# jyjblrd/Low-Cost-Mocap

Measured on AMD Instinct MI355X. Metric: triangulated 3D markers/sec at 8 cams x 16 markers, higher is better.
Workload: dtype f64

## Files before the change

### low-cost-mocap_amd/csrc/capi.hip

```cpp
#include <hip/hip_runtime.h>

#include <cmath>
#include <cstdarg>
#include <cstdio>
#include <cstdlib>
#include <cstring>
#include <mutex>
#include <string>
#include <vector>

#include "../../include/mocap_core.h"
#include "ctx.hpp"

using namespace mocap;

int mocap_ctx::fail(int code, const char* fmt, ...) {
  char buf[512];
  va_list ap;
  va_start(ap, fmt);
  vsnprintf(buf, sizeof buf, fmt, ap);
  va_end(ap);
  {
    std::lock_guard<std::mutex> lk(err_mu);
    err = buf;
// ... 29 lines not shown
  cap = want;
  return 0;
}

hipError_t PinBuf::reserve(size_t need, size_t want, unsigned flags) {
  if (need <= cap) return hipSuccess;
  if (ptr) (void)hipHostFree(ptr);
  ptr = nullptr;
  cap = 0;
  const hipError_t e = hipHostMalloc(&ptr, want, flags);
  if (e == hipSuccess) cap = want;
  return e;
}

int spin_wait(mocap_ctx* ctx, Event& event) {
  HIP_TRY(ctx, event.ready());
  HIP_TRY(ctx, hipEventRecord(event.ev, ctx->stream));
  for (long spins = 0;; spins++) {
    const hipError_t e = hipEventQuery(event.ev);
    if (e == hipSuccess) return MOCAP_OK;
    if (e != hipErrorNotReady) return ctx->hip_fail(e, "hipEventQuery");
    if (spins > 2000000) {
      HIP_TRY(ctx, hipStreamSynchronize(ctx->stream));
      return MOCAP_OK;
    }
  }
}

extern "C" int mocap_create(int device_id, mocap_ctx** out) {
  if (!out) return MOCAP_E_ARG;
  *out = nullptr;
  int ndev = 0;
  if (hipGetDeviceCount(&ndev) != hipSuccess || device_id < 0 || device_id >= ndev) return MOCAP_E_HIP;
  mocap_ctx* c = new mocap_ctx();
  c->device = device_id;
  if (hipSetDevice(device_id) != hipSuccess || hipStreamCreate(&c->own_stream) != hipSuccess) {
    delete c;
    return MOCAP_E_HIP;
  }
  c->stream = c->own_stream;
  hipDeviceProp_t prop;
  if (hipGetDeviceProperties(&prop, device_id) == hipSuccess) c->num_cus = prop.multiProcessorCount;
  const char* t = getenv("MOCAP_FRAME_THREADS");
  if (t) {
    int v = atoi(t);
    if (v == 64 || v == 128 || v == 256) c->frame_threads = v;
  }
  if ((t = getenv("MOCAP_HEAVY_THRESHOLD"))) c->heavy_threshold = atoi(t);
  if ((t = getenv("MOCAP_SLICE_SIZE"))) c->slice_size = atoi(t);
  if ((t = getenv("MOCAP_FORCE_WIDE"))) c->force_wide = atoi(t) ? 1 : 0;
  if ((t = getenv("MOCAP_PRUNE"))) c->prune = atoi(t) ? 1 : 0;
  if ((t = getenv("MOCAP_EIGCUT"))) c->eigcut = atoi(t) ? 1 : 0;
  if ((t = getenv("MOCAP_EVAL_BB"))) c->eval_bb = atoi(t) ? 1 : 0;
  if ((t = getenv("MOCAP_BB_PL")) && atoi(t) >= 1 && atoi(t) <= 64) c->bb_pl = atoi(t);
  if ((t = getenv("MOCAP_BB_FLUSH")) && atoi(t) >= 1) c->bb_flush = atoi(t);
  if ((t = getenv("MOCAP_BB_MIN_G")) && atoi(t) >= 0) c->bb_min_g = atoi(t);
  if ((t = getenv("MOCAP_FRAME_LAUNCHES"))) c->frame_launches = atoi(t) == 3 ? 3 : 1;
  *out = c;
  return MOCAP_OK;
}

extern "C" void mocap_destroy(mocap_ctx* ctx) {
  if (!ctx) return;
  (void)hipSetDevice(ctx->device);
  (void)hipStreamSynchronize(ctx->stream);
  if (ctx->own_stream) (void)hipStreamDestroy(ctx->own_stream);
  delete ctx;
}

extern "C" const char* mocap_last_error(const mocap_ctx* ctx) {
  if (!ctx) return "null context";
  static thread_local std::string mine;
  {
    std::lock_guard<std::mutex> lk(const_cast<mocap_ctx*>(ctx)->err_mu);
    mine = ctx->err;
  }
  return mine.c_str();
}
extern "C" const char* mocap_version(void) { return "mocap_core 0.1 (gfx950)"; }

extern "C" int mocap_set_stream(mocap_ctx* ctx, void* hip_stream) {
  if (!ctx) return MOCAP_E_ARG;
  std::lock_guard<std::mutex> lk(ctx->mu);
  hipStream_t ns = hip_stream ? (hipStream_t)hip_stream : ctx->own_stream;
  if (ns != ctx->stream && ctx->dev_outstanding) {
    int prev_dev = -1;
    (void)hipGetDevice(&prev_dev);
    HIP_TRY(ctx, hipSetDevice(ctx->device));
    const hipError_t e = hipStreamWaitEvent(ns, ctx->handover_event.ev, 0);
    if (prev_dev >= 0 && prev_dev != ctx->device) (void)hipSetDevice(prev_dev);
    if (e != hipSuccess) return ctx->hip_fail(e, "hipStreamWaitEvent(handover)");
    ctx->frame_q_dirty();
  }
  ctx->stream = ns;
  return MOCAP_OK;
}

extern "C" const char* mocap_last_frame_kernel(mocap_ctx* ctx) {
  if (!ctx) return "none";
  std::lock_guard<std::mutex> lk(ctx->mu);
  return ctx->last_frame_kernel;
}

extern "C" int mocap_synchronize(mocap_ctx* ctx) {
  if (!ctx) return MOCAP_E_ARG;
  std::lock_guard<std::mutex> lk(ctx->mu);
  HIP_TRY(ctx, hipSetDevice(ctx->device));
// ... 413 lines not shown
```

### low-cost-mocap_amd/csrc/ctx.hpp

```cpp
#pragma once
#include <hip/hip_runtime.h>

#include <mutex>
#include <string>
#include <vector>

#include "kernels.hpp"

#define HIP_TRY(ctx, expr)                                     \
  do {                                                         \
    hipError_t e__ = (expr);                                   \
    if (e__ != hipSuccess) return (ctx)->hip_fail(e__, #expr); \
  } while (0)

struct Owned {
  Owned() = default;
  Owned(const Owned&) = delete;
};

struct DevBuf : Owned {
  void* ptr = nullptr;
  size_t cap = 0;
  int reserve(size_t bytes);
  ~DevBuf() { if (ptr) (void)hipFree(ptr); }
};

struct PinBuf : Owned {
  void* ptr = nullptr;
  size_t cap = 0;
  hipError_t reserve(size_t need, size_t want, unsigned flags);
  ~PinBuf() { if (ptr) (void)hipHostFree(ptr); }
};

struct Event : Owned {
  hipEvent_t ev = nullptr;
  hipError_t ready() { return ev ? hipSuccess : hipEventCreateWithFlags(&ev, hipEventDisableTiming); }
  ~Event() { if (ev) (void)hipEventDestroy(ev); }
};

struct Carver {
  uintptr_t base;
  size_t align, off = 0;
  explicit Carver(void* b, size_t align_ = 256) : base((uintptr_t)b), align(align_) {}
  template <class T>
  static size_t padded(size_t count, size_t align = 256) { return (sizeof(T) * count + align - 1) / align * align; }
  template <class T>
  T* take(size_t count) {
    T* p = (T*)(base + off);
    off += padded<T>(count, align);
    return p;
  }
  void align_to(size_t a) { off = (off + a - 1) / a * a; }
};

struct mocap_ctx {
  int device = 0;
  int num_cus = 256;
  int frame_threads = 0;
  int heavy_threshold = -1;
  int slice_size = 0;
  int hit_cap = 32;
  int force_wide = 0;
  int32_t frame_gen = 0;
  int frame_q_cap[2] = {0, 0};
  const char* last_frame_kernel = "none";
  bool frame_q_clean[2] = {false, false};
  void frame_q_dirty() { frame_q_clean[0] = frame_q_clean[1] = false; }
  int frame_launches = 1;
  int prune = 1;
  int exhaustive = 0;
  int eval_bb = 1;
  int bb_pl = 16;
  int bb_min_g = 0;
  int bb_flush = 0;
  int eigcut = 1;
  double eig_c0[3] = {0, 0, 0};
  double p3max2c = 0.0;
  double p3max2 = 0.0;
  hipStream_t own_stream = nullptr, stream = nullptr;
  Event handover_event;
  bool dev_outstanding = false;
  int mark_enqueued();
  std::mutex mu;
  std::string err;
  std::mutex err_mu;
  uint32_t flags = 1u;
  int C = 0;
  std::vector<double> hK, hR, ht, hF;
  DevBuf tables;
  const double* d_K9 = nullptr;
  mocap::CamView cv{};
  PinBuf ba_pin;
  Event ba_event;
  PinBuf ba_stage;
  void (*ba_progress)(const double* x, int n, void* user) = nullptr;
  void* ba_progress_user = nullptr;
  DevBuf ba_fused;
  double ba_stamp = 0.0;
  PinBuf live_pin;
  Event live_event;
  DevBuf world;
  bool world_on = false;
  int img_C = 0, img_rows = 0, img_cols = 0, img_S = 0, img_ay = 0;
  DevBuf img_map, img_rot, img_mask, img_stage, img_tiles, img_lens, img_fix, img_fixidx, img_act, img_box, img_zero;
  int img_n_lt = 0;
  int blob_skip_dark = 1;
  int centroid_mode = 0;
  DevBuf img_grey, img_bbox;
  DevBuf compact_ws;
  DevBuf frame_ws;
  DevBuf bb_ws;
  DevBuf live_stage;
  DevBuf resub;
  DevBuf resub_ctr;
  DevBuf resub_q;
  DevBuf heavy_recs;
  DevBuf heavy_ws;
  DevBuf heavy_enum;
  uint32_t resub_calls = 0;
  DevBuf scratch[4];
  int objf_D = 0, objf_B = 0;
  float objf_q = 0.f, objf_r = 0.f;
  DevBuf objf_state;
  DevBuf objf_ws;
  uint32_t objf_calls = 0;
// ... 59 lines not shown
```

### low-cost-mocap_amd/csrc/frame_bb.hip

```cpp
#include "mocap_device.hpp"
#include "kernels.hpp"
#include <cstdlib>
#include "frame_common.hpp"

namespace mocap {

constexpr int kBBThreads = 256;
constexpr int kBBWaves = kBBThreads / 64;
constexpr int kBBRecs = kBBThreads + 64;
constexpr int bb_cw(int C) { return C <= 8 ? 1 : 2; }
constexpr uint32_t bb_rec_bytes(int CW) { return 24u + 8u * (uint32_t)CW; }

constexpr int bb_wg_per_cu(int RL) { return RL == 48 ? 5 : 4; }
constexpr int kBBLdsSlack = 1024;
struct BBLayout {
  size_t bxy, bxy_nx, cnt_nx, bt, rbound, seedkey, slot_key, claimw, recs, rpk, scr, scr_bytes, goff, gcnt, outslot, boff, bnb, seedgh, slot_g, cnt,
      misc, bpl, nh, hits, act, root_blob, root_cam, nact, bnl, bv, bcache, bpk, total;
  int ncache;
  __host__ __device__ static size_t al(size_t x, size_t a) { return (x + a - 1) / a * a; }
  __host__ __device__ BBLayout(int C, int M, int R, int CW, int wg_per_cu) {
    size_t o = 0;
    auto take = [&](size_t bytes, size_t a) {
      o = al(o, a);
      const size_t at = o;
      o += bytes;
      return at;
    };
    bxy = take(sizeof(float2) * (size_t)C * M, 16);
    bxy_nx = take(sizeof(float2) * (size_t)C * M, 16);
    cnt_nx = take(4 * (size_t)C, 4);
    bt = take(sizeof(double) * 10 * ((size_t)C * M + 1), 16);
    rbound = take(8 * (size_t)R, 8);
    claimw = take(8 * (size_t)C, 8);
    scr = seedkey = take(8 * (size_t)R, 8);
    slot_key = take(8 * (size_t)kBBWaves * R, 8);
    recs = take(8 * (size_t)kBBRecs, 8);
    rpk = take(8 * (size_t)kBBRecs * CW, 8);
    seedgh = take(4 * (size_t)R, 4);
    slot_g = take(4 * (size_t)kBBWaves * R, 4);
    scr_bytes = o - scr;
    goff = take(4 * (size_t)(R + 1), 4);
    gcnt = take(4 * (size_t)R, 4);
    outslot = take(4 * (size_t)R, 4);
    boff = take(4 * (size_t)(R + 1), 4);
    bnb = take(4 * (size_t)R, 4);
    cnt = take(4 * (size_t)C, 4);
    misc = take(4 * 16, 4);
    bpl = take(2 * (size_t)R, 2);
    nh = take((size_t)R * C, 1);
    hits = take((size_t)R * C * M, 1);
    act = take((size_t)R * C, 1);
    root_blob = take((size_t)R, 1);
    root_cam = take((size_t)R, 1);
    nact = take((size_t)R, 1);
    bnl = take((size_t)R, 1);
    bv = take((size_t)R, 1);
    bcache = take(0, 8);
    ncache = 0;
    const size_t per_entry = 8 + 8 * (size_t)CW;
    for (int per_cu = wg_per_cu; per_cu >= 1; per_cu--) {
      const size_t lim = ((size_t)160 * 1024 / per_cu - kBBLdsSlack) / 256 * 256;
      if (lim >= o + per_entry * 64) {
        const size_t n = (lim - o) / per_entry;
        ncache = (int)(n > 1024 ? 1024 : n);
        break;
      }
    }
    o += 8 * (size_t)ncache;
    bpk = o;
    o += 8 * (size_t)CW * ncache;
    total = al(o, 16);
  }
};

static int bb_fixed_slots(int C, int M, int R) {
  const char* e = getenv("MOCAP_BB_FIXED_LAYOUT");
  if (e && e[0] == '0') return 0;
  if (C == 8 && M == 16 && R <= 48) return 48;
  if (C == 8 && M == 16 && R <= 64) return 64;
  return 0;
}
static int frame_bb_root_slots(int C, int M, int R) {
  const int f = bb_fixed_slots(C, M, R);
  return f ? f : R;
}
size_t frame_bb_lds_bytes(int C, int M, int R) { return BBLayout(C, M, frame_bb_root_slots(C, M, R), bb_cw(C), bb_wg_per_cu(bb_fixed_slots(C, M, R))).total; }
static size_t frame_bb_lds_bytes_min(int C, int M, int R) {
  const BBLayout L(C, M, frame_bb_root_slots(C, M, R), bb_cw(C), bb_wg_per_cu(bb_fixed_slots(C, M, R)));
  return L.total - (8 + 8 * (size_t)bb_cw(C)) * (size_t)L.ncache;
}
bool frame_bb_fits(int C, int M, int R) {
  return C >= 2 && C <= 16 && M >= 1 && M <= 64 && R >= 1 && R <= 255 && frame_bb_lds_bytes_min(C, M, R) <= (size_t)128 * 1024;
}

template <int CW>
struct Packed {
  unsigned long long w[CW];
  __device__ __forceinline__ void clear() {
#pragma unroll
    for (int k = 0; k < CW; k++) w[k] = ~0ull;
  }
  __device__ __forceinline__ void set(int c, uint32_t idx) {
    if (CW == 1)
      w[0] ^= (unsigned long long)(idx ^ 0xFFu) << (8 * c);
    else
      w[c >> 3] ^= (unsigned long long)(idx ^ 0xFFu) << (8 * (c & 7));
  }
  __device__ __forceinline__ uint32_t get(int c) const {
    return CW == 1 ? (uint32_t)(w[0] >> (8 * c)) & 0xFFu : (uint32_t)(w[c >> 3] >> (8 * (c & 7))) & 0xFFu;
  }
};

template <int CT, bool PERK = false>
struct BBCamTables {
  const double* base;
  static constexpr int C = CT;
  static constexpr int kPq = PERK ? 12 * CT * CT : 12 * CT;
  __device__ __forceinline__ ctab_t pq(size_t off) const { return as_ctab(base + off); }
  __device__ __forceinline__ ctab_t rt(size_t off) const { return as_ctab(base + kPq + off); }
  __device__ __forceinline__ ctab_t k4(size_t off) const { return as_ctab(base + kPq + 12 * CT + off); }
  __device__ __forceinline__ const double* f() const { return base + kPq + 16 * CT; }
};
template <bool PERK>
struct BBCamTables<0, PERK> {
  const double* base;
  int C;
  __device__ __forceinline__ ctab_t pq(size_t off) const { return as_ctab(base + off); }
  __device__ __forceinline__ ctab_t rt(size_t off) const { return as_ctab(base + (PERK ? 12 * C * C : 12 * C) + off); }
  __device__ __forceinline__ ctab_t k4(size_t off) const { return as_ctab(base + (PERK ? 12 * C * C + 12 * C : 24 * C) + off); }
  __device__ __forceinline__ const double* f() const { return base + (PERK ? 12 * C * C + 16 * C : 28 * C); }
};

enum { kPrioEval = 0, kPrioSeed = 1, kPrioPhase = 2, kPrioSerial = 3 };
template <int P>
__device__ __forceinline__ void bb_prio() {
  __builtin_amdgcn_s_setprio(P);
}

template <bool F32R, int CW, int CT, int ML, int RL, bool PERK = false>
struct BBState {
  static constexpr int T = kBBThreads, W = kBBWaves;
  const FrameArgs& p;
  BBCamTables<CT, PERK> cv;
  const int C_, M, R, RS;
  int tid, lane, wave;
  __device__ __forceinline__ void fresh_tid() {
    int t = tid;
    asm volatile("" : "+v"(t));
    tid = t;
    lane = t & 63;
    wave = t >> 6;
  }
  __device__ __forceinline__ int cn() const { return CT > 0 ? CT : C_; }
  double* bt;
  float2 *bxy, *bxy_nx;
  int32_t* cnt_nx;
  unsigned long long *rbound, *seedkey, *slot_key, *claimw, *rpk;
  struct BRec { uint32_t gh, rs; };
  BRec* recs;
  uint32_t *goff, *gcnt, *boff, *bnb, *seedgh, *slot_g;
  int32_t *outslot, *cnt, *misc;
  uint16_t* bpl;
  uint8_t *nh, *hits, *act, *root_blob, *root_cam, *nact, *bnl, *bv;
  float2* bcache;
  unsigned long long* bpk;
  int ncache;
  unsigned char* scr;
  size_t scr_bytes;
  static constexpr unsigned long long kInfBits = 0x7ff0000000000000ull;

  __device__ BBState(const FrameArgs& p_, unsigned char* smem)
      : p(p_), C_(p_.cv.C), M(ML > 0 ? ML : p_.M), R(p_.K_max), RS(RL > 0 ? RL : p_.K_max), tid(threadIdx.x), lane(threadIdx.x & 63), wave(threadIdx.x >> 6) {
    const int C = cn();
    {
      const unsigned long long ta = (unsigned long long)(uintptr_t)p_.cv.Pq;
      uint32_t tlo = (uint32_t)__builtin_amdgcn_readfirstlane((int)(uint32_t)ta);
      uint32_t thi = (uint32_t)__builtin_amdgcn_readfirstlane((int)(uint32_t)(ta >> 32));
      asm volatile("" : "+s"(tlo), "+s"(thi));
      cv.base = (const double*)(uintptr_t)(((unsigned long long)thi << 32) | tlo);
      if constexpr (CT == 0) cv.C = C;
    }
    const BBLayout L(C, M, RS, CW, bb_wg_per_cu(RL));
    bt = (double*)(smem + L.bt);
    bxy = (float2*)(smem + L.bxy);
    bxy_nx = (float2*)(smem + L.bxy_nx);
    cnt_nx = (int32_t*)(smem + L.cnt_nx);
    rbound = (unsigned long long*)(smem + L.rbound);
    seedkey = (unsigned long long*)(smem + L.seedkey);
    slot_key = (unsigned long long*)(smem + L.slot_key);
    claimw = (unsigned long long*)(smem + L.claimw);
    recs = (BRec*)(smem + L.recs);
    rpk = (unsigned long long*)(smem + L.rpk);
    goff = (uint32_t*)(smem + L.goff);
    gcnt = (uint32_t*)(smem + L.gcnt);
    outslot = (int32_t*)(smem + L.outslot);
    boff = (uint32_t*)(smem + L.boff);
    bnb = (uint32_t*)(smem + L.bnb);
    seedgh = (uint32_t*)(smem + L.seedgh);
    slot_g = (uint32_t*)(smem + L.slot_g);
    cnt = (int32_t*)(smem + L.cnt);
    misc = (int32_t*)(smem + L.misc);
    bpl = (uint16_t*)(smem + L.bpl);
    nh = (uint8_t*)(smem + L.nh);
    hits = (uint8_t*)(smem + L.hits);
    act = (uint8_t*)(smem + L.act);
    root_blob = (uint8_t*)(smem + L.root_blob);
    root_cam = (uint8_t*)(smem + L.root_cam);
    nact = (uint8_t*)(smem + L.nact);
    bnl = (uint8_t*)(smem + L.bnl);
    bv = (uint8_t*)(smem + L.bv);
    scr = smem + L.scr;
    scr_bytes = L.scr_bytes;
    bcache = (float2*)(smem + L.bcache);
    bpk = (unsigned long long*)(smem + L.bpk);
    ncache = L.ncache;
  }

  struct Line { double a, b, c, den, rden; };
  __device__ __forceinline__ Line epiline(int r, int i) const { return epiline_of(root_cam[r], root_blob[r], i); }
  __device__ __forceinline__ Line epiline_of(int rc, int rb, int i) const {
    const int C = cn();
    const double* Fm = cv.f() + 9 * ((size_t)rc * C + i);
    const float2 rp = bxy[(size_t)rc * M + rb];
    const double x = (double)rp.x, y = (double)rp.y;
    double a = Fm[0] * x + Fm[1] * y + Fm[2];
    double b = Fm[3] * x + Fm[4] * y + Fm[5];
    double c = Fm[6] * x + Fm[7] * y + Fm[8];
    double nu = a * a + b * b;
    nu = nu != 0.0 ? 1.0 / sqrt(nu) : 1.0;
    a *= nu;
    b *= nu;
    c *= nu;
    if (F32R) {
      a = (double)(float)a;
      b = (double)(float)b;
      c = (double)(float)c;
    }
    Line L;
    L.a = a;
    L.b = b;
    L.c = c;
    L.den = sqrt(a * a + b * b);
    L.rden = recip_refined(L.den);
    return L;
  }

  template <bool CHAIN>
  __device__ __forceinline__ unsigned long long match_pairs(const Line& mine, int pair_r, int pair_i, int n_pairs, int gs_shift,
                                                            int cam = 0, int Mi_chain = 0) {
    const int C = cn();
    const int GS = 1 << gs_shift, PPS = 64 >> gs_shift;
    const int k = lane & (GS - 1), q = lane >> gs_shift;
    const int gl0 = lane & ~(GS - 1);
    const unsigned long long gall = gs_shift == 6 ? ~0ull : ((1ull << GS) - 1ull);
    unsigned long long claims = 0ull;
    for (int s0 = 0; s0 < n_pairs; s0 += PPS) {
      const int src = s0 + q;
      const bool has = src < n_pairs;
      const int sl = has ? src : 0;
      const double la = __shfl(mine.a, sl), lb = __shfl(mine.b, sl), lc = __shfl(mine.c, sl);
      const double lden = __shfl(mine.den, sl), lrden = __shfl(mine.rden, sl);
      const int r = __shfl(pair_r, sl);
      const int i = CHAIN ? cam : __shfl(pair_i, sl);
      const int Mi = has ? (CHAIN ? Mi_chain : cnt[i]) : 0;
      const bool valid = k < Mi;
      float2 pt = make_float2(0.f, 0.f);
      double d = 0.0;
// ... 327 lines not shown
        if (n_roots > R) {
          over = true;
          n_roots = R;
        }
      }
      if (lane == 0) {
        if (over) misc[MI_STATUS] |= MOCAP_ST_ROOT_OVERFLOW_;
        misc[MI_NROOTS] = n_roots;
      }
    } else {
      float om = 0.0f;
      for (int i = tid - 64; i < C * M; i += T - 64) {
        const int c = i / M, k = i - c * M;
        if (k < cnt[c]) {
          const float2 v = bxy[i];
          om = fmaxf(om, fmaxf(fabsf(v.x), fabsf(v.y)));
          double Bc[10];
          dlt_contribution(Bc, cv.pq(PERK ? 12 * (c * C + c) : 12 * c), (double)v.x, (double)v.y);
#pragma unroll
          for (int e = 0; e < 10; e++) bt[(size_t)i * 10 + e] = Bc[e];
        }
      }
      if (om > 0.0f) atomicMax(&misc[MI_OMAX], __float_as_int(om));
      if (tid == 64) {
        const int it = q_add(&p.q.counters[QC_NEXT_FRAME], 1);
        misc[MI_NEXT] = it < frame_count(p) ? it : -1;
      }
    }
    bb_prio<kPrioPhase>();
    __syncthreads();
    if (pre) {
      const int n_new = misc[MI_NROOTS] - n0;
      for (int idx = tid; idx < n_new * C; idx += T) {
        const int q = idx / C, c = idx - q * C;
        const int r = n0 + q, ps = bnl[q];
        if (c > (int)root_cam[r]) {
          const int n = nh_s[(size_t)ps * C + c];
          nh[(size_t)r * C + c] = (uint8_t)n;
          const uint8_t* src = hits_s + ((size_t)ps * C + c) * M;
          uint8_t* dst = hits + ((size_t)r * C + c) * M;
          for (int t = 0; t < n; t++) dst[t] = src[t];
        }
      }
      __syncthreads();
    }

    fresh_tid();
    const int nroots = misc[MI_NROOTS];
    for (int r = tid; r < nroots; r += T) {
      const int rc = root_cam[r];
      unsigned long long total = 1;
      int views = 1, na = 0;
      bool over = false;
      for (int c = rc + 1; c < C; c++) {
        const unsigned n = nh[(size_t)r * C + c];
        if (n > 1) act[(size_t)r * C + na++] = (uint8_t)c;
        if (n) {
          views++;
          total *= n;
          if (total > (unsigned long long)p.G_cap) {
            over = true;
            total = 1;
          }
        }
      }
      if (over) atomicOr(&misc[MI_STATUS], MOCAP_ST_CAND_OVERFLOW_);
      nact[r] = (uint8_t)na;
      bv[r] = (uint8_t)views;
      rbound[r] = kInfBits;
      const uint32_t g = (views > 1 && !over) ? (uint32_t)total : 0u;
      gcnt[r] = g;
      {
        const uint8_t* a = act + (size_t)r * C;
        uint32_t pl = 1, nb = 1;
        int nl = 0;
        while (nl < na && pl < (uint32_t)p.bb_pl) pl *= nh[(size_t)r * C + a[nl++]];
        for (int k = nl; k < na; k++) nb *= nh[(size_t)r * C + a[k]];
        bpl[r] = (uint16_t)pl;
        bnl[r] = (uint8_t)nl;
        bnb[r] = g ? nb : 0u;
        seedkey[r] = 0ull;
        seedgh[r] = 0xFFFFFFFFu;
      }
    }
    for (int s = tid; s < W * RS; s += T) {
      slot_key[s] = ~0ull;
      slot_g[s] = 0xFFFFFFFFu;
    }
    if (tid == 0) misc[MI_BBCTR] = misc[MI_BBCTR2] = 0;
    __syncthreads();
    if (wave == 0) bb_prio<kPrioSerial>();
    if (wave == 0) {
      uint32_t carry = 0, bcarry = 0;
      int slots = 0;
      for (int base = 0; base < nroots; base += 64) {
        const int r = base + lane;
        const uint32_t g = r < nroots ? gcnt[r] : 0u;
        const uint32_t nb = r < nroots ? bnb[r] : 0u;
        const uint32_t incl = wave_inclusive_scan(g, lane);
        const uint32_t bincl = wave_inclusive_scan(nb, lane);
        const unsigned long long nz = __ballot(g != 0u);
        if (r < nroots) {
          goff[r] = carry + incl - g;
          boff[r] = bcarry + bincl - nb;
          outslot[r] = g ? slots + __popcll(nz & ((1ull << lane) - 1ull)) : -1;
        }
        carry += (uint32_t)__builtin_amdgcn_readlane((int)incl, 63);
        bcarry += (uint32_t)__builtin_amdgcn_readlane((int)bincl, 63);
        slots += __popcll(nz);
      }
      if (lane == 0) {
        goff[nroots] = carry;
        boff[nroots] = bcarry;
        misc[MI_NOUT] = slots;
        misc[MI_G] = misc[MI_STATUS] ? 0 : (int32_t)carry;
      }
    }
    bb_prio<kPrioPhase>();
    __syncthreads();
  }

  __device__ __forceinline__ void add_view(double (&B)[10], int c, uint32_t k, int j) const {
    if (PERK && j != c) {
      const float2 w = bxy[(size_t)c * M + k];
      double Bc[10];
      dlt_contribution(Bc, cv.base + 12 * ((size_t)j * cn() + c), (double)w.x, (double)w.y);
#pragma unroll
      for (int e = 0; e < 10; e++) B[e] = B[e] + Bc[e];
    } else {
      const double* t = bt + ((size_t)c * M + k) * 10;
#pragma unroll
      for (int e = 0; e < 10; e++) B[e] = B[e] + t[e];
    }
  }

  template <bool WITH_B>
  __device__ __forceinline__ int group_matrix(int r, uint32_t rem, int skip, double (&B)[10], Packed<CW>& pk) const {
    const int C = cn();
    const int rc = root_cam[r];
    const uint8_t* nhr = nh + (size_t)r * C;
    const uint8_t* hr = hits + (size_t)r * C * M;
    pk.clear();
    int v = 0, ka = 0;
    int j = 0;
    if (WITH_B) {
#pragma unroll
      for (int e = 0; e < 10; e++) B[e] = 0.0;
    }
    for (int c = 0; c < C; c++) {
      uint32_t k = 0xFFu;
      bool seen = false;
      if (c == rc) {
        k = root_blob[r];
        seen = true;
      } else if (c > rc) {
        const uint32_t n = nhr[c];
        seen = n != 0;
        if (n == 1) {
          k = hr[(size_t)c * M];
        } else if (n > 1) {
          if (ka >= skip) {
            uint32_t qd, dgt;
            if (rem < 8192u) divmod_tiny(rem, n, qd, dgt); else
            divmod_small(rem, n, qd, dgt);
            rem = qd;
            k = hr[(size_t)c * M + dgt];
          }
          ka++;
        }
      }
      if (k != 0xFFu) {
        if (WITH_B) add_view(B, c, k, j);
        v++;
        pk.set(c, k);
      }
      if (PERK) j += seen ? 1 : 0;
    }
    return v;
  }

  __device__ __forceinline__ int fetch_candidate(uint32_t lo, uint32_t i, int& r, uint32_t& gl, Packed<CW>& pk, double (&B)[10]) const {
    const int C = cn();
    const BRec rec = recs[lo];
    r = (int)(rec.rs & 0xFFu);
#pragma unroll
    for (int k = 0; k < CW; k++) pk.w[k] = rpk[(size_t)lo * CW + k];
    if (rec.rs >> 31) {
      gl = rec.gh;
    } else {
      uint32_t rem = i - (rec.rs >> 8);
      gl = rec.gh * (uint32_t)bpl[r] + rem;
      const uint8_t* a = act + (size_t)r * C;
      const int nl = bnl[r];
      for (int k = 0; k < nl; k++) {
        const int c = a[k];
        uint32_t qd, dgt;
        divmod_tiny(rem, nh[(size_t)r * C + c], qd, dgt);
        rem = qd;
        pk.set(c, hits[((size_t)r * C + c) * M + dgt]);
      }
    }
#pragma unroll
    for (int ee = 0; ee < 10; ee++) B[ee] = 0.0;
    if constexpr (PERK) {
      int j = 0;
#pragma unroll CT > 0 ? CT : 1
      for (int c = 0; c < C; c++) {
        const uint32_t k = pk.get(c);
        if (k != 0xFFu) add_view(B, c, k, j++);
      }
    } else {
#pragma unroll CT > 0 ? CT : 1
      for (int c = 0; c < C; c++) {
        const uint32_t k = pk.get(c);
        const double* t = bt + (size_t)(k != 0xFFu ? (uint32_t)c * (uint32_t)M + k : (uint32_t)C * (uint32_t)M) * 10;
#pragma unroll
        for (int ee = 0; ee < 10; ee++) B[ee] = B[ee] + t[ee];
      }
    }
    return bv[r];
  }

  __device__ void search(bool bound_tests) {
    fresh_tid();
    const int C = cn();
    (void)C;
    const int nroots = misc[MI_NROOTS];
    int32_t* ctr = &misc[MI_BBCTR];
    int32_t* ctr_other = &misc[MI_BBCTR2];
    const double inf = __builtin_huge_val();
    EigCut ec;
    {
      const double om = (double)__int_as_float(misc[MI_OMAX]);
      ec.p3max2 = p.p3max2;
      ec.o2slack = (1100.0 * 0x1p-46) * (om * om);
    }
    const double c0[3] = {p.bb_c0[0], p.bb_c0[1], p.bb_c0[2]};
    const uint32_t nblocks = boff[nroots];
    auto root_of_block = [&](uint32_t b_first_of_wave, uint32_t b) {
      return coop_last_le([&](int r) { return boff[r]; }, nroots, b_first_of_wave, b, lane);
    };
    auto push_block = [&](int r, uint32_t gh, const Packed<CW>& pk) {
      const uint32_t old = (uint32_t)atomicAdd(ctr, (int32_t)(((uint32_t)bpl[r] << 10) | 1u));
      const uint32_t slot = old & 0x3FFu;
      BRec rec;
      rec.gh = gh;
      rec.rs = (uint32_t)r | ((old >> 10) << 8);
      recs[slot] = rec;
#pragma unroll
      for (int k = 0; k < CW; k++) rpk[(size_t)slot * CW + k] = pk.w[k];
    };
    auto rec_start = [&](int k) { return (recs[k].rs & 0x7FFFFFFFu) >> 8; };
    auto dropped = [&](int r, double s1, double tr) {
      const int vf = bv[r];
      const double bound = __longlong_as_double((long long)rbound[r]);
      const double limit = bound * (double)(2 * vf) * (1.0 + 0x1p-40);
      const double limit_adj = fma(1.002, limit, (double)(2 * vf) * ec.o2slack);
      return s1 * fma(2e-12, tr, p.p3max2c * limit_adj) < 1.0;
    };
    if (bound_tests) {
      bb_prio<kPrioSeed>();
      int my_r = -1;
      uint32_t my_gh = 0;
      unsigned long long my_key = 0ull;
      Packed<CW> my_pk;
      my_pk.clear();
      for (uint32_t s0 = 0; s0 < nblocks; s0 += T) {
        const uint32_t b = s0 + (uint32_t)tid;
        if (s0 + (uint32_t)(wave * 64) >= nblocks) continue;
        const int r = root_of_block(s0 + (uint32_t)(wave * 64), b < nblocks ? b : nblocks - 1);
        if (b < nblocks) {
          const uint32_t gh = b - boff[r];
          double B[10], tr = 0.0;
          Packed<CW> pk;
          const int v = group_matrix<true>(r, gh, bnl[r], B, pk);
          double s1d = __builtin_huge_val();
          float s1 = 0.0f;
          if (v >= 2) {
            s1d = eigcut_s1_shifted(B, c0, tr);
            s1 = (float)fmin(s1d, 3e38);
          }
          if (b < (uint32_t)ncache) {
            bcache[b] = make_float2(__double2float_ru(s1d), __double2float_ru(tr));
#pragma unroll
            for (int k = 0; k < CW; k++) bpk[(size_t)b * CW + k] = pk.w[k];
          }
          my_key = ((unsigned long long)__float_as_uint(s1) << 32) | (unsigned long long)(0xFFFFFFFFu - gh);
          my_r = r;
          my_gh = gh;
          my_pk = pk;
          atomicMax(&seedkey[r], my_key);
        }
      }
      __syncthreads();
      if (nblocks <= (uint32_t)T) {
        if (my_r >= 0 && seedkey[my_r] == my_key) {
          seedgh[my_r] = my_gh;
          push_block(my_r, my_gh, my_pk);
        }
      } else
      for (int r = tid; r < nroots; r += T) {
        if (bnb[r]) {
          const uint32_t gh = 0xFFFFFFFFu - (uint32_t)seedkey[r];
          seedgh[r] = gh;
          seedkey[r] = 0ull;
          double B[10];
          Packed<CW> pk;
          group_matrix<false>(r, gh, bnl[r], B, pk);
          push_block(r, gh, pk);
        }
      }
      bb_prio<kPrioEval>();
      __syncthreads();
    }
    uint32_t b0 = 0;
    fresh_tid();
    while (true) {
      const uint32_t cv_ = (uint32_t)*ctr;
      const uint32_t ns = cv_ & 0x3FFu, ne = cv_ >> 10;
      const bool blocks_left = b0 < nblocks;
      const bool full = ns > (uint32_t)(kBBRecs - T);
      if (ns && (full || !blocks_left || ne >= (uint32_t)p.bb_flush)) {
        for (uint32_t i0 = 0; i0 < ne; i0 += T) {
          const uint32_t i = i0 + (uint32_t)tid;
          const bool have = i < ne;
          double e = inf, X[3] = {0, 0, 0};
          int r = 0;
          uint32_t gl = 0;
          uint32_t lo = 0;
          if (i0 + (uint32_t)(wave * 64) < ne)
            lo = (uint32_t)coop_last_le(rec_start, (int)ns, i0 + (uint32_t)(wave * 64), have ? i : ne - 1, lane);
          Packed<CW> pk;
          pk.clear();
          if (have) {
            double B[10];
            const int v = fetch_candidate(lo, i, r, gl, pk, B);
            auto obs_p = [&](int c, double& x, double& y) -> bool {
              const uint32_t k = pk.get(c);
              if (k == 0xFFu) return false;
              const float2 w = bxy[(size_t)c * M + k];
              x = (double)w.x;
              y = (double)w.y;
              return true;
            };
            const double bound = __longlong_as_double((long long)rbound[r]);
            solve_and_score<!PERK, true, F32R, false>(cv, B, v, obs_p, X, e, bound * (double)(2 * v) * (1.0 + 0x1p-40), ec);
#ifdef MOCAP_DEBUG_EIGCHECK
            if (!(e < inf)) {
              double B2[10], X2[3], e2;
#pragma unroll
              for (int ee = 0; ee < 10; ee++) B2[ee] = 0.0;
              int j2 = 0;
              for (int c = 0; c < C; c++) {
                const uint32_t k = pk.get(c);
                if (k != 0xFFu) add_view(B2, c, k, j2++);
              }
              solve_and_score<!PERK, true, F32R>(cv, B2, v, obs_p, X2, e2);
              atomicAdd(&p.status[p.n_frames], 1);
              if (e2 <= bound) printf("EIGCHECK candidate: root %d g %u bound %.17g true %.17g\n", r, gl, bound, e2);
            }
#endif
          }
          const bool fin = e < inf;
          const unsigned long long key = fin ? (unsigned long long)__double_as_longlong(e) : kInfBits;
          const uint32_t gword = (gl << 1) | ((e != e) ? 1u : 0u);
          const int ss = wave * RS + r;
          if (fin) atomicMin(&rbound[r], key);
          const bool want = have && (key < slot_key[ss] || (key == slot_key[ss] && gword < slot_g[ss]));
          if (__ballot(want)) {
            unsigned long long old = 0;
            if (want) old = atomicMin(&slot_key[ss], key);
            wave_lds_sync();
            const bool holder = want && slot_key[ss] == key;
            if (holder && old > key) slot_g[ss] = 0xFFFFFFFFu;
            wave_lds_sync();
            if (holder) atomicMin(&slot_g[ss], gword);
            wave_lds_sync();
            if (holder && slot_g[ss] == gword) store_winner(ss, X, pk);
          }
        }
        __syncthreads();
        if (tid == 0) *ctr = 0;
        {
          int32_t* t = ctr;
          ctr = ctr_other;
          ctr_other = t;
        }
        continue;
      }
      if (!blocks_left) break;
      const uint32_t b = b0 + (uint32_t)tid;
      const uint32_t bw = b0 + (uint32_t)(wave * 64);
      b0 += T;
      int r = 0;
      if (bw < nblocks) r = root_of_block(bw, b < nblocks ? b : nblocks - 1);
      bool do_push = false;
      uint32_t gh = 0;
      Packed<CW> pk;
      pk.clear();
      if (b < nblocks) {
        gh = b - boff[r];
        if (gh != seedgh[r]) {
          double B[10], tr;
          bool survive = true;
          if (bound_tests && b < (uint32_t)ncache) {
            const float2 sc = bcache[b];
            survive = !dropped(r, (double)sc.x, (double)sc.y);
#pragma unroll
            for (int k = 0; k < CW; k++) pk.w[k] = bpk[(size_t)b * CW + k];
          } else if (bound_tests) {
            const int v = group_matrix<true>(r, gh, bnl[r], B, pk);
            if (v >= 2) {
              const double s1 = eigcut_s1_shifted(B, c0, tr);
              survive = !dropped(r, s1, tr);
            }
          } else {
            group_matrix<false>(r, gh, bnl[r], B, pk);
          }
          do_push = survive;
#ifdef MOCAP_DEBUG_EIGCHECK
          if (!survive) {
            const double bound = __longlong_as_double((long long)rbound[r]);
            const uint32_t pl = bpl[r];
            for (uint32_t l = 0; l < pl; l++) {
              double B2[10], X2[3], e2 = inf;
              Packed<CW> pk2;
              const int v2 = group_matrix<true>(r, gh * pl + l, 0, B2, pk2);
              auto obs2 = [&](int c, double& x, double& y) -> bool {
                const uint32_t k = pk2.get(c);
                if (k == 0xFFu) return false;
                const float2 w = bxy[(size_t)c * M + k];
                x = (double)w.x;
                y = (double)w.y;
                return true;
              };
              solve_and_score<!PERK, true, F32R>(cv, B2, v2, obs2, X2, e2);
              atomicAdd(&p.status[p.n_frames + 1], 1);
              if (e2 <= bound) printf("EIGCHECK block: root %d block %u candidate %u bound %.17g true %.17g\n", r, gh, l, bound, e2);
            }
          }
#endif
        }
      }
      __syncthreads();
      if (do_push) push_block(r, gh, pk);
      __syncthreads();
    }
    wait_own_stores();
    __syncthreads();
  }

  __device__ __forceinline__ bool root_winner(int r, unsigned long long& kb, uint32_t& gw, int& wb) const {
    kb = ~0ull;
    gw = 0xFFFFFFFFu;
    wb = 0;
    for (int w = 0; w < W; w++) {
      const int s = w * RS + r;
      const unsigned long long k = slot_key[s];
      const uint32_t g = slot_g[s];
      if (k < kb || (k == kb && g < gw)) {
        kb = k;
        gw = g;
        wb = w;
      }
    }
    return kb != ~0ull;
  }

  static constexpr uint32_t kRecBytes = bb_rec_bytes(CW);
  __device__ __forceinline__ unsigned char* winner_rec(int s) const {
// ... 101 lines not shown
```

### low-cost-mocap_amd/csrc/frame_capi.hip

```cpp
#include <hip/hip_runtime.h>

#include <cstdlib>
#include <cstring>
#include <mutex>
#include <stdexcept>
#include <vector>

#include "../../include/mocap_core.h"
#include "ctx.hpp"
#include "jpeg_tables.hpp"

using namespace mocap;

namespace {

struct FrameBatch {
  int64_t n_frames;
  int M_max;
  const float* blobs;
  const int32_t* counts;
  double gate_px;
};
struct FrameOut {
  double* xyz;
// ... 41 lines not shown
    const char* wt = getenv("MOCAP_WIDE_THREADS");
    const size_t l2 = frame_lds(ctx, M_max, K_max, 512, pl.hit_cap, true);
    if (!(wt && atoi(wt) == 1024) && 2 * l2 <= kLdsBytes && ctx->frame_launches != 3) {
      pl.T = 512;
      pl.lds = l2;
    }
  }
  return pl;
}

bool frame_shape_fits(const mocap_ctx* ctx, int M_max, int K) {
  if (frame_bb_fits(ctx->C, M_max, K) && (ctx->cv.uniformK || ctx->p3max2 > 0.0) && !ctx->force_wide && M_max <= 255) return true;
  if (!must_go_wide(ctx, M_max) && frame_lds(ctx, M_max, K, 64, M_max, false) <= kLdsBytes) return true;
  return frame_lds(ctx, M_max, K, kWideThreads, M_max, true) <= kLdsBytes;
}

struct HeavyHook {
  int32_t* count;
  unsigned char* recs;
  int cap;
};

FrameArgs frame_args(const mocap_ctx* ctx, const FrameBatch& b, int K_max, int64_t G_cap, const FrameOut& o,
                     const FramePlan& pl, const int32_t* n_frames_dev, const HeavyHook* heavy) {
  const int M_max = b.M_max;
  FrameArgs a;
  a.cv = ctx->cv;
  a.n_frames = b.n_frames;
  a.n_frames_dev = n_frames_dev;
  a.M = M_max;
  a.K_max = K_max;
  a.gate_px = b.gate_px;
  a.G_cap = G_cap;
  a.blobs = b.blobs;
  a.counts = b.counts;
  a.xyz = o.xyz;
  a.err = o.err;
  a.corr = o.corr;
  a.n_out = o.n_out;
  a.status = o.status;
  a.n_cand = o.n_cand;
  a.world = ctx->world_on ? (const double*)ctx->world.ptr : nullptr;
  a.H = pl.hit_cap;
  a.wide = pl.wide ? 1 : 0;
  if (pl.wide) {
    const char* sp = getenv("MOCAP_WIDE_SPEC");
    if (sp && atoi(sp) == 0) a.wide = 2;
  }
  a.prune = ctx->prune && !ctx->exhaustive;
  a.p3max2 = a.prune && ctx->eigcut ? ctx->p3max2 : 0.0;
  if (!pl.wide && ctx->frame_threads == 0 && pl.T == 64) a.p3max2 = 0.0;
  a.eval_bb = pl.use_bb ? 1 : 0;
  a.bb_pl = ctx->bb_pl;
  for (int i = 0; i < 3; i++) a.bb_c0[i] = ctx->eig_c0[i];
  a.p3max2c = ctx->p3max2c;
  a.bb_flush = ctx->bb_flush > 0 ? ctx->bb_flush : 256;
  a.bb_min_g = ctx->bb_min_g;
  while (a.bb_pl > 1 && (size_t)a.bb_pl * M_max * 2 * 256 >= ((size_t)1 << 22)) a.bb_pl /= 2;
  a.ws = nullptr;
  a.ws_stride = 0;
  const bool hv = heavy && pl.wide;
  a.heavy_bb = hv ? 1 : 0;
  a.heavy_cap = hv ? heavy->cap : 0;
  a.heavy_count = hv ? heavy->count : nullptr;
  a.heavy_recs = hv ? heavy->recs : nullptr;
  a.heavy_stride = hv ? heavy_rec_bytes(ctx->C, pl.hit_cap) : 0;
  return a;
}

size_t lay_queues(FrameQueues& q, void* base, int K_max) {
  Carver c(base);
  q.counters = c.take<int32_t>(QC_COUNT);
  q.slice_heavy = c.take<int32_t>(q.W_cap);
  q.slice_gen = c.take<int32_t>(q.W_cap);
  q.heavy = c.take<int32_t>(4 * (size_t)q.H_cap);
  q.part_e = c.take<double>((size_t)q.W_cap * K_max);
  q.part_g = c.take<uint32_t>((size_t)q.W_cap * K_max);
  q.part_x = c.take<double>(3 * (size_t)q.W_cap * K_max);
  return c.off;
}

int prepare_queues(mocap_ctx* ctx, FrameArgs& a, const FramePlan& pl, int64_t full_grid, bool one_launch) {
  const int64_t n_frames = a.n_frames;
  const bool batch = n_frames >= 2 * full_grid;
  FrameQueues& q = a.q;
  q.heavy_threshold = ctx->heavy_threshold >= 0 ? (uint32_t)ctx->heavy_threshold : (batch ? 32768u : 16u * pl.T);
  q.slice_size = ctx->slice_size > 0 ? (uint32_t)ctx->slice_size : (batch ? (pl.wide ? 24576u : 8192u) : 4u * pl.T);
  if (a.heavy_bb) q.heavy_threshold = 0;
  q.frame_chunk = 1;
  if (ctx->C * a.M <= 32) {
    int64_t ch = n_frames / (full_grid * 64);
    q.frame_chunk = (int)(ch < 1 ? 1 : (ch > 16 ? 16 : ch));
  }
  int64_t H = n_frames / 8;
  if (H < 64) H = 64;
  if (H > n_frames) H = n_frames;
  q.H_cap = (int)H;
  q.W_cap = (int)(H * 8 < 64 ? 64 : H * 8);
  const int qs = a.n_frames_dev ? 1 : 0;
  DevBuf& wq = qs ? ctx->resub_q : ctx->scratch[3];
  const void* wq_before = wq.ptr;
  if (wq.reserve(lay_queues(q, nullptr, a.K_max))) return ctx->fail(MOCAP_E_HIP, "hipMalloc(frame work queues) failed");
  lay_queues(q, wq.ptr, a.K_max);
  const bool fresh = wq.ptr != wq_before || ctx->frame_q_cap[qs] != q.W_cap || !ctx->frame_q_clean[qs];
  q.gen = ++ctx->frame_gen;
  if (ctx->frame_gen == 0x7fffffff) {
    ctx->frame_gen = 0;
    ctx->frame_q_dirty();
  }
  if ((!one_launch && !pl.use_bb) || fresh) {
    const size_t b_slice = Carver::padded<int32_t>(q.W_cap);
// ... 829 lines not shown
```

### low-cost-mocap_amd/csrc/kernels.hpp

```cpp
#pragma once
#include <hip/hip_runtime.h>
#include <stdint.h>

#include "mocap_device.hpp"

namespace mocap {

constexpr int MOCAP_ST_ROOT_OVERFLOW_ = 1;
constexpr int MOCAP_ST_CAND_OVERFLOW_ = 2;
constexpr int MOCAP_ST_HIT_OVERFLOW_ = 4;
constexpr int MOCAP_ST_INTRACTABLE_ = 16;
constexpr int MOCAP_ST_FINAL_ = 32;
constexpr int MOCAP_ST_LOG2_GROUPS_SHIFT_ = 20;

constexpr int MODE_MAIN = 0, MODE_SLICE = 1, MODE_MERGE = 2, MODE_ALL = 3;
enum { QC_NEXT_FRAME = 0, QC_N_HEAVY = 1, QC_N_SLICES = 2, QC_NEXT_SLICE = 3, QC_NEXT_MERGE = 4, QC_FRAMES_DONE = 5, QC_EXITED = 6, QC_COUNT = 8 };
struct FrameQueues {
  int32_t* counters;
  int32_t* heavy;
  int32_t* slice_heavy;
  int32_t* slice_gen;
  int32_t gen;
  double* part_e;
  uint32_t* part_g;
  double* part_x;
  int H_cap, W_cap;
  uint32_t heavy_threshold;
  uint32_t slice_size;
  int frame_chunk;
};

struct FrameArgs {
  CamView cv;
  FrameQueues q;
  int64_t n_frames;
  int M;
  int K_max;
  double gate_px;
  int64_t G_cap;
  const float* blobs;
  const int32_t* counts;
  double* xyz;
  double* err;
  int16_t* corr;
  int32_t* n_out;
  int32_t* status;
  int32_t* n_cand;
  const double* world;
  unsigned char* ws;
  size_t ws_stride;
  int H;
  int wide;
  int prune;
  int eval_bb;
  int bb_pl;
  int bb_flush;
  int bb_min_g;
  double bb_c0[3];
  double p3max2c;
  double p3max2;
  const int32_t* n_frames_dev;
  int heavy_bb;
  int heavy_cap;
  int32_t* heavy_count;
  unsigned char* heavy_recs;
  size_t heavy_stride;
};

struct HeavyRecHdr {
  int32_t frame, root, outslot, rc, rb, omax_bits, views, Hs;
};
__host__ __device__ inline size_t heavy_rec_counts_off() { return sizeof(HeavyRecHdr); }
__host__ __device__ inline size_t heavy_rec_hits_off(int C) { return (sizeof(HeavyRecHdr) + 2 * (size_t)C + 15) / 16 * 16; }
__host__ __device__ inline size_t heavy_rec_bytes(int C, int Hs) { return (heavy_rec_hits_off(C) + (size_t)C * Hs + 15) / 16 * 16; }

struct HeavyArgs {
  CamView cv;
  int M, K_big;
  double bb_c0[3], p3max2c, p3max2;
  const float* blobs;
  const int32_t* heavy_count;
  const unsigned char* recs;
  int cap;
  size_t stride;
  double* xyz;
  double* err;
  int16_t* corr;
  int32_t* n_out;
  int32_t* status;
  const double* world;
  unsigned char* ws;
  size_t ws_stride;
  int ncap;
  int64_t enum_cap;
  int debug;
  int32_t* enum_count;
  int32_t* enum_list;
  int32_t* enum_slice;
  int32_t* enum_done;
  unsigned long long* enum_bound;
  unsigned char* enum_part;
  int enum_max, enum_grid;
};
constexpr int kHeavyEnumPartBytes = 40;
constexpr int kHeavyEnumMax = 256;
hipError_t launch_heavy_enum(const HeavyArgs& a, hipStream_t stream);
size_t heavy_bb_ws_bytes(int ncap);
hipError_t launch_heavy_bb(const HeavyArgs& a, int grid, hipStream_t stream);
// ... 350 lines not shown
```

Baseline: 589.8 million.

## Shrink branch-and-bound block cache to folded float bounds and rebuild packs on demand

Replaces the per-block LDS cache, which held an (s1, tr) float pair plus the full packed candidate, with a single conservatively rounded float bound. The packed candidate is rebuilt only for surviving blocks, from a per-root base pack plus digit decoding (block_pk/block_matrix). This frees LDS so more blocks can be cached. It also adds an adaptive block-split rule (bb_pl_min / bb_nb_max) that chooses how many active cameras go into each block. The cost is extra recomputation of packs and a slightly looser, rounded pruning bound.

```diff
diff --git a/low-cost-mocap_amd/csrc/bb_fold.hpp b/low-cost-mocap_amd/csrc/bb_fold.hpp
--- /dev/null
+++ b/low-cost-mocap_amd/csrc/bb_fold.hpp
@@ -0,0 +1,43 @@
+#pragma once
+#include <cmath>
+#include <cstdint>
+#include <cstring>
+
+#if defined(__HIPCC__) || defined(__CUDACC__)
+#define BB_FOLD_FN __host__ __device__ inline
+#else
+#define BB_FOLD_FN inline
+#endif
+
+namespace mocap {
+
+BB_FOLD_FN float bb_fold_inf() {
+  const uint32_t u = 0x7f800000u;
+  float f;
+  memcpy(&f, &u, 4);
+  return f;
+}
+
+BB_FOLD_FN float bb_fold_float_up(double x) {
+  float f = (float)x;
+  if ((double)f < x) {
+    uint32_t u;
+    memcpy(&u, &f, 4);
+    u += 1u;
+    memcpy(&f, &u, 4);
+  }
+  return f;
+}
+
+BB_FOLD_FN float bb_fold_bound(double s1, double tr) {
+  const double den = 1.0 - s1 * (2e-12 * tr);
+  if (!(den > 0x1p-20) || !(s1 == s1)) return bb_fold_inf();
+  const double q = (s1 / den) * (1.0 + 0x1p-20);
+  if (!(q < 3e38)) return bb_fold_inf();
+  if (!(q > 0x1p-126)) return s1 > 0.0 ? 0x1p-126f : (float)q;
+  return bb_fold_float_up(q);
+}
+
+BB_FOLD_FN bool bb_fold_dropped(float q, double y) { return (double)q * y < 1.0; }
+
+}
diff --git a/low-cost-mocap_amd/csrc/capi.hip b/low-cost-mocap_amd/csrc/capi.hip
--- a/low-cost-mocap_amd/csrc/capi.hip
+++ b/low-cost-mocap_amd/csrc/capi.hip
@@ -105,7 +105,10 @@
   if ((t = getenv("MOCAP_PRUNE"))) c->prune = atoi(t) ? 1 : 0;
   if ((t = getenv("MOCAP_EIGCUT"))) c->eigcut = atoi(t) ? 1 : 0;
   if ((t = getenv("MOCAP_EVAL_BB"))) c->eval_bb = atoi(t) ? 1 : 0;
-  if ((t = getenv("MOCAP_BB_PL")) && atoi(t) >= 1 && atoi(t) <= 64) c->bb_pl = atoi(t);
+  if ((t = getenv("MOCAP_BB_PL_MIN")) && atoi(t) >= 1 && atoi(t) <= 64) c->bb_pl_min = atoi(t);
+  if ((t = getenv("MOCAP_BB_NB_MAX")) && atoi(t) >= 1) c->bb_nb_max = atoi(t);
+  if (c->bb_pl_min > c->bb_pl) c->bb_pl_min = c->bb_pl;
+  if ((t = getenv("MOCAP_BB_PL")) && atoi(t) >= 1 && atoi(t) <= 64) c->bb_pl = c->bb_pl_min = atoi(t);
   if ((t = getenv("MOCAP_BB_FLUSH")) && atoi(t) >= 1) c->bb_flush = atoi(t);
   if ((t = getenv("MOCAP_BB_MIN_G")) && atoi(t) >= 0) c->bb_min_g = atoi(t);
   if ((t = getenv("MOCAP_FRAME_LAUNCHES"))) c->frame_launches = atoi(t) == 3 ? 3 : 1;
diff --git a/low-cost-mocap_amd/csrc/ctx.hpp b/low-cost-mocap_amd/csrc/ctx.hpp
--- a/low-cost-mocap_amd/csrc/ctx.hpp
+++ b/low-cost-mocap_amd/csrc/ctx.hpp
@@ -71,6 +71,8 @@
   int exhaustive = 0;
   int eval_bb = 1;
   int bb_pl = 16;
+  int bb_pl_min = 16;
+  int bb_nb_max = 1;
   int bb_min_g = 0;
   int bb_flush = 0;
   int eigcut = 1;
diff --git a/low-cost-mocap_amd/csrc/frame_bb.hip b/low-cost-mocap_amd/csrc/frame_bb.hip
--- a/low-cost-mocap_amd/csrc/frame_bb.hip
+++ b/low-cost-mocap_amd/csrc/frame_bb.hip
@@ -2,6 +2,7 @@
 #include "kernels.hpp"
 #include <cstdlib>
 #include "frame_common.hpp"
+#include "bb_fold.hpp"
 
 namespace mocap {
 
@@ -12,10 +13,11 @@
 constexpr uint32_t bb_rec_bytes(int CW) { return 24u + 8u * (uint32_t)CW; }
 
 constexpr int bb_wg_per_cu(int RL) { return RL == 48 ? 5 : 4; }
+constexpr size_t kBBCacheEntry = 4;
 constexpr int kBBLdsSlack = 1024;
 struct BBLayout {
   size_t bxy, bxy_nx, cnt_nx, bt, rbound, seedkey, slot_key, claimw, recs, rpk, scr, scr_bytes, goff, gcnt, outslot, boff, bnb, seedgh, slot_g, cnt,
-      misc, bpl, nh, hits, act, root_blob, root_cam, nact, bnl, bv, bcache, bpk, total;
+      misc, bpl, nh, hits, act, root_blob, root_cam, nact, bnl, bv, pkbase, seen, bcache, total;
   int ncache;
   __host__ __device__ static size_t al(size_t x, size_t a) { return (x + a - 1) / a * a; }
   __host__ __device__ BBLayout(int C, int M, int R, int CW, int wg_per_cu) {
@@ -32,6 +34,7 @@
     bt = take(sizeof(double) * 10 * ((size_t)C * M + 1), 16);
     rbound = take(8 * (size_t)R, 8);
     claimw = take(8 * (size_t)C, 8);
+    pkbase = take(8 * (size_t)CW * R, 8);
     scr = seedkey = take(8 * (size_t)R, 8);
     slot_key = take(8 * (size_t)kBBWaves * R, 8);
     recs = take(8 * (size_t)kBBRecs, 8);
@@ -47,6 +50,7 @@
     cnt = take(4 * (size_t)C, 4);
     misc = take(4 * 16, 4);
     bpl = take(2 * (size_t)R, 2);
+    seen = take(2 * (size_t)R, 2);
     nh = take((size_t)R * C, 1);
     hits = take((size_t)R * C * M, 1);
     act = take((size_t)R * C, 1);
@@ -55,9 +59,9 @@
     nact = take((size_t)R, 1);
     bnl = take((size_t)R, 1);
     bv = take((size_t)R, 1);
-    bcache = take(0, 8);
+    bcache = take(0, 4);
     ncache = 0;
-    const size_t per_entry = 8 + 8 * (size_t)CW;
+    const size_t per_entry = kBBCacheEntry;
     for (int per_cu = wg_per_cu; per_cu >= 1; per_cu--) {
       const size_t lim = ((size_t)160 * 1024 / per_cu - kBBLdsSlack) / 256 * 256;
       if (lim >= o + per_entry * 64) {
@@ -66,9 +70,7 @@
         break;
       }
     }
-    o += 8 * (size_t)ncache;
-    bpk = o;
-    o += 8 * (size_t)CW * ncache;
+    o += per_entry * (size_t)ncache;
     total = al(o, 16);
   }
 };
@@ -87,7 +89,7 @@
 size_t frame_bb_lds_bytes(int C, int M, int R) { return BBLayout(C, M, frame_bb_root_slots(C, M, R), bb_cw(C), bb_wg_per_cu(bb_fixed_slots(C, M, R))).total; }
 static size_t frame_bb_lds_bytes_min(int C, int M, int R) {
   const BBLayout L(C, M, frame_bb_root_slots(C, M, R), bb_cw(C), bb_wg_per_cu(bb_fixed_slots(C, M, R)));
-  return L.total - (8 + 8 * (size_t)bb_cw(C)) * (size_t)L.ncache;
+  return L.total - kBBCacheEntry * (size_t)L.ncache;
 }
 bool frame_bb_fits(int C, int M, int R) {
   return C >= 2 && C <= 16 && M >= 1 && M <= 64 && R >= 1 && R <= 255 && frame_bb_lds_bytes_min(C, M, R) <= (size_t)128 * 1024;
@@ -162,8 +164,9 @@
   int32_t *outslot, *cnt, *misc;
   uint16_t* bpl;
   uint8_t *nh, *hits, *act, *root_blob, *root_cam, *nact, *bnl, *bv;
-  float2* bcache;
-  unsigned long long* bpk;
+  float* bcache;
+  unsigned long long* pkbase;
+  uint16_t* seen;
   int ncache;
   unsigned char* scr;
   size_t scr_bytes;
@@ -211,8 +214,9 @@
     bv = (uint8_t*)(smem + L.bv);
     scr = smem + L.scr;
     scr_bytes = L.scr_bytes;
-    bcache = (float2*)(smem + L.bcache);
-    bpk = (unsigned long long*)(smem + L.bpk);
+    bcache = (float*)(smem + L.bcache);
+    pkbase = (unsigned long long*)(smem + L.pkbase);
+    seen = (uint16_t*)(smem + L.seen);
     ncache = L.ncache;
   }
 
@@ -646,10 +650,16 @@
       unsigned long long total = 1;
       int views = 1, na = 0;
       bool over = false;
+      Packed<CW> pkb;
+      pkb.clear();
+      pkb.set(rc, root_blob[r]);
+      uint32_t sm = 1u << rc;
       for (int c = rc + 1; c < C; c++) {
         const unsigned n = nh[(size_t)r * C + c];
         if (n > 1) act[(size_t)r * C + na++] = (uint8_t)c;
+        if (n == 1) pkb.set(c, hits[((size_t)r * C + c) * M]);
         if (n) {
+          sm |= 1u << c;
           views++;
           total *= n;
           if (total > (unsigned long long)p.G_cap) {
@@ -661,6 +671,9 @@
       if (over) atomicOr(&misc[MI_STATUS], MOCAP_ST_CAND_OVERFLOW_);
       nact[r] = (uint8_t)na;
       bv[r] = (uint8_t)views;
+#pragma unroll
+      for (int k = 0; k < CW; k++) pkbase[(size_t)r * CW + k] = pkb.w[k];
+      if (PERK) seen[r] = (uint16_t)sm;
       rbound[r] = kInfBits;
       const uint32_t g = (views > 1 && !over) ? (uint32_t)total : 0u;
       gcnt[r] = g;
@@ -668,8 +681,14 @@
         const uint8_t* a = act + (size_t)r * C;
         uint32_t pl = 1, nb = 1;
         int nl = 0;
-        while (nl < na && pl < (uint32_t)p.bb_pl) pl *= nh[(size_t)r * C + a[nl++]];
-        for (int k = nl; k < na; k++) nb *= nh[(size_t)r * C + a[k]];
+        for (int k = 0; k < na; k++) nb *= nh[(size_t)r * C + a[k]];
+        if (over) nb = 1;
+        while (nl < na && (pl < (uint32_t)p.bb_pl_min || (pl < (uint32_t)p.bb_pl && nb > (uint32_t)p.bb_nb_max))) {
+          const uint32_t n = nh[(size_t)r * C + a[nl++]];
+          uint32_t dummy;
+          pl *= n;
+          divmod_small(nb, n, nb, dummy);
+        }
         bpl[r] = (uint16_t)pl;
         bnl[r] = (uint8_t)nl;
         bnb[r] = g ? nb : 0u;
@@ -773,6 +792,47 @@
     return v;
   }
 
+  __device__ __forceinline__ void block_pk(int r, uint32_t gh, Packed<CW>& pk) const {
+    const int C = cn();
+#pragma unroll
+    for (int k = 0; k < CW; k++) pk.w[k] = pkbase[(size_t)r * CW + k];
+    const uint8_t* a = act + (size_t)r * C;
+    const int na = nact[r];
+    uint32_t rem = gh;
+    for (int k = bnl[r]; k < na; k++) {
+      const int c = a[k];
+      const uint32_t n = nh[(size_t)r * C + c];
+      uint32_t qd, dgt;
+      if (rem < 8192u) divmod_tiny(rem, n, qd, dgt); else
+      divmod_small(rem, n, qd, dgt);
+      rem = qd;
+      pk.set(c, hits[((size_t)r * C + c) * M + dgt]);
+    }
+  }
+  __device__ __forceinline__ int block_matrix(int r, uint32_t gh, Packed<CW>& pk, double (&B)[10]) const {
+    const int C = cn();
+    block_pk(r, gh, pk);
+#pragma unroll
+    for (int ee = 0; ee < 10; ee++) B[ee] = 0.0;
+    if constexpr (PERK) {
+      const uint32_t sm = seen[r];
+#pragma unroll CT > 0 ? CT : 1
+      for (int c = 0; c < C; c++) {
+        const uint32_t k = pk.get(c);
+        if (k != 0xFFu) add_view(B, c, k, __popc(sm & ((1u << c) - 1u)));
+      }
+    } else {
+#pragma unroll CT > 0 ? CT : 1
+      for (int c = 0; c < C; c++) {
+        const uint32_t k = pk.get(c);
+        const double* t = bt + (size_t)(k != 0xFFu ? (uint32_t)c * (uint32_t)M + k : (uint32_t)C * (uint32_t)M) * 10;
+#pragma unroll
+        for (int ee = 0; ee < 10; ee++) B[ee] = B[ee] + t[ee];
+      }
+    }
+    return (int)bv[r] - (int)bnl[r];
+  }
+
   __device__ __forceinline__ int fetch_candidate(uint32_t lo, uint32_t i, int& r, uint32_t& gl, Packed<CW>& pk, double (&B)[10]) const {
     const int C = cn();
     const BRec rec = recs[lo];
@@ -845,13 +905,14 @@
       for (int k = 0; k < CW; k++) rpk[(size_t)slot * CW + k] = pk.w[k];
     };
     auto rec_start = [&](int k) { return (recs[k].rs & 0x7FFFFFFFu) >> 8; };
-    auto dropped = [&](int r, double s1, double tr) {
+    auto root_y = [&](int r) {
       const int vf = bv[r];
       const double bound = __longlong_as_double((long long)rbound[r]);
       const double limit = bound * (double)(2 * vf) * (1.0 + 0x1p-40);
       const double limit_adj = fma(1.002, limit, (double)(2 * vf) * ec.o2slack);
-      return s1 * fma(2e-12, tr, p.p3max2c * limit_adj) < 1.0;
+      return p.p3max2c * limit_adj;
     };
+    auto dropped = [&](int r, double s1, double tr) { return s1 * fma(2e-12, tr, root_y(r)) < 1.0; };
     if (bound_tests) {
       bb_prio<kPrioSeed>();
       int my_r = -1;
@@ -867,18 +928,14 @@
           const uint32_t gh = b - boff[r];
           double B[10], tr = 0.0;
           Packed<CW> pk;
-          const int v = group_matrix<true>(r, gh, bnl[r], B, pk);
+          const int v = block_matrix(r, gh, pk, B);
           double s1d = __builtin_huge_val();
           float s1 = 0.0f;
           if (v >= 2) {
             s1d = eigcut_s1_shifted(B, c0, tr);
             s1 = (float)fmin(s1d, 3e38);
           }
-          if (b < (uint32_t)ncache) {
-            bcache[b] = make_float2(__double2float_ru(s1d), __double2float_ru(tr));
-#pragma unroll
-            for (int k = 0; k < CW; k++) bpk[(size_t)b * CW + k] = pk.w[k];
-          }
+          if (b < (uint32_t)ncache) bcache[b] = v >= 2 ? bb_fold_bound(s1d, tr) : bb_fold_inf();
           my_key = ((unsigned long long)__float_as_uint(s1) << 32) | (unsigned long long)(0xFFFFFFFFu - gh);
           my_r = r;
           my_gh = gh;
@@ -898,9 +955,8 @@
           const uint32_t gh = 0xFFFFFFFFu - (uint32_t)seedkey[r];
           seedgh[r] = gh;
           seedkey[r] = 0ull;
-          double B[10];
           Packed<CW> pk;
-          group_matrix<false>(r, gh, bnl[r], B, pk);
+          block_pk(r, gh, pk);
           push_block(r, gh, pk);
         }
       }
@@ -998,18 +1054,16 @@
           double B[10], tr;
           bool survive = true;
           if (bound_tests && b < (uint32_t)ncache) {
-            const float2 sc = bcache[b];
-            survive = !dropped(r, (double)sc.x, (double)sc.y);
-#pragma unroll
-            for (int k = 0; k < CW; k++) pk.w[k] = bpk[(size_t)b * CW + k];
+            survive = !bb_fold_dropped(bcache[b], root_y(r));
+            if (survive) block_pk(r, gh, pk);
           } else if (bound_tests) {
-            const int v = group_matrix<true>(r, gh, bnl[r], B, pk);
+            const int v = block_matrix(r, gh, pk, B);
             if (v >= 2) {
               const double s1 = eigcut_s1_shifted(B, c0, tr);
               survive = !dropped(r, s1, tr);
             }
           } else {
-            group_matrix<false>(r, gh, bnl[r], B, pk);
+            block_pk(r, gh, pk);
           }
           do_push = survive;
 #ifdef MOCAP_DEBUG_EIGCHECK
diff --git a/low-cost-mocap_amd/csrc/frame_capi.hip b/low-cost-mocap_amd/csrc/frame_capi.hip
--- a/low-cost-mocap_amd/csrc/frame_capi.hip
+++ b/low-cost-mocap_amd/csrc/frame_capi.hip
@@ -117,11 +117,13 @@
   if (!pl.wide && ctx->frame_threads == 0 && pl.T == 64) a.p3max2 = 0.0;
   a.eval_bb = pl.use_bb ? 1 : 0;
   a.bb_pl = ctx->bb_pl;
+  a.bb_nb_max = ctx->bb_nb_max;
   for (int i = 0; i < 3; i++) a.bb_c0[i] = ctx->eig_c0[i];
   a.p3max2c = ctx->p3max2c;
   a.bb_flush = ctx->bb_flush > 0 ? ctx->bb_flush : 256;
   a.bb_min_g = ctx->bb_min_g;
   while (a.bb_pl > 1 && (size_t)a.bb_pl * M_max * 2 * 256 >= ((size_t)1 << 22)) a.bb_pl /= 2;
+  a.bb_pl_min = ctx->bb_pl_min < a.bb_pl ? ctx->bb_pl_min : a.bb_pl;
   a.ws = nullptr;
   a.ws_stride = 0;
   const bool hv = heavy && pl.wide;
diff --git a/low-cost-mocap_amd/csrc/kernels.hpp b/low-cost-mocap_amd/csrc/kernels.hpp
--- a/low-cost-mocap_amd/csrc/kernels.hpp
+++ b/low-cost-mocap_amd/csrc/kernels.hpp
@@ -54,6 +54,7 @@
   int prune;
   int eval_bb;
   int bb_pl;
+  int bb_pl_min, bb_nb_max;
   int bb_flush;
   int bb_min_g;
   double bb_c0[3];
```

New measurement: 598.8 million (median of 6 runs). 1.02x the previous value.
